# YuePanEdward/MULLS

Measured on NVIDIA H100. Metric: scan-pair registrations/sec (120k-pt 64-beam), higher is better.
Workload: dtype f32 geometry / f64 accumulation

## Files before the change

### mulls_b200/csrc/device_types.cuh

```cuda
#pragma once
#include <cstdint>
#include <cuda_runtime.h>

#include "../../include/mulls_b200/abi.h"
#include "search_core.cuh"

namespace mulls {

constexpr int kNumClasses = MULLS_NUM_CLASSES;
constexpr int kNumSegs = 2 * kNumClasses;
constexpr int kIterBlock = 128;
constexpr int kIngestBlock = 256;
constexpr int kTerms = 28;
constexpr int kMaxLevels = 12;
constexpr int kCoordBits = 12;
constexpr int kDedupMinSrc = 500;
constexpr unsigned kClaimFree = 0x7f7f7f7fu;
constexpr int kIterFlags = 256;

enum PairStatus : int { kRunning = 0, kNeedPosterior = 1, kDone = 2 };

struct ChunkDesc {
    uint32_t pair;
    uint32_t seg;
// ... 18 lines not shown
    int normal_shooting;
    int keep_less;
    uint32_t random_seed;
    double cos_thre;
    double sigma_thre;
    double init[16];
    double tbound[6];
    uint32_t in_off[kNumSegs];
    const float4 *in_ptr[kNumSegs];
    uint32_t in_n[kNumSegs];
    uint32_t in_fmt[kNumSegs];
    uint32_t tgt_base[kNumClasses];
    uint32_t src_base[kNumClasses];
    uint32_t chunk_begin;
    uint32_t chunk_end;
    uint32_t class_chunk_begin[kNumClasses + 1];
    uint32_t src_index_base[kNumClasses];
    uint32_t src_global_n[kNumClasses];
    int sharded;
};

struct PairState {
    double T_total[16];
    double T_inc[16];
    double x[6];
    double cofactor[36];
    double info[36];
    double sigma2;
    double ibb[6];
    float thre;
    float confidence;
    float origin[3];
    float h0, inv_h0;
    int n_levels;
    int status, code, iter, iters_entered, final_buf;
    int source_feature_points_count;
    int n_src[kNumClasses];
    int n_src_g[kNumClasses];
    int n_src_g_next[kNumClasses];
    int n_tgt[kNumClasses];
    uint32_t n_corr[kNumClasses];
    uint32_t n_corr_last[kNumClasses];
    uint32_t seg_count[kNumSegs];
    uint32_t seg_start[kNumSegs];
    uint32_t hash_entries[kNumClasses];
    uint32_t hash_base[kNumClasses];
    uint32_t hash_mask[kNumClasses];
    int bb_src[6];
    int bb_tgt[6];
    uint64_t alg_bytes;
    int kl_keep[kNumSegs];
    uint32_t kl_rank[kNumSegs];
    uint64_t kl_prefix[kNumSegs];
    uint32_t kl_hist[kNumSegs][256];
};

struct LoopCtl {
    int it;
    int n_it_chunks;
    int n_pairs;
    int trace_on;
    int max_iter;
    unsigned solved;
    unsigned n_live[2];
    unsigned work[4];
};

struct DeviceArrays {
    const float4 *in_aos;
    uint64_t *keys_a, *keys_b;
    uint32_t *vals_a, *vals_b;
    float4 *tgt_pos, *tgt_nrm;
    float4 *src_pos[2], *src_nrm[2];
    int *src_prevj[2];
    float4 *src_cert[2];
    int *nn_idx;
    float *nn_d2;
    uint8_t *flags;
    int *corr_j;
    float *corr_w;
    unsigned *claim;
    HashEntry *hash;
    uint32_t hash_pool_entries;
    uint32_t *hash_used;
    uint32_t *blk_kept;
    double *partials;
    double *post_partials;
    PairConst *pc;
    PairState *ps;
    ChunkDesc *in_chunks;
    ChunkDesc *it_chunks;
    mulls_icp_trace *trace;
    int *xch_i32;
    double *xch_f64;
    LoopCtl *ctl;
    uint32_t *live_chunks;
    uint32_t live_stride;
    int *running;
    volatile int *h_running;
    volatile int *h_running_iter;
};

}
```

### mulls_b200/csrc/grid_key.cuh

```cuda
#pragma once
#include <cstdint>

#ifdef __CUDACC__
#define MULLS_HD __host__ __device__ __forceinline__
#else
#define MULLS_HD inline
#endif

namespace mulls {

constexpr uint32_t kKeyHiMask = 0xffffu;

MULLS_HD float flann_l2(float px, float py, float pz, float qx, float qy, float qz) {
    const float dx = px - qx, dy = py - qy, dz = pz - qz;
    return (dx * dx + dy * dy) + dz * dz;
}

MULLS_HD uint32_t cell_key_lo(uint32_t x, uint32_t y, uint32_t z) { return x | (y << 12) | ((z & 0xffu) << 24); }
MULLS_HD uint32_t cell_key_hi(uint32_t z, int level) { return (z >> 8) | ((uint32_t)(level + 1) << 4); }

MULLS_HD uint32_t cell_hash(uint32_t klo, uint32_t khi) {
    uint32_t h = klo * 0x9E3779B1u;
    h ^= khi * 0x85EBCA77u;
    h ^= h >> 15;
    h *= 0x2C1B3C6Du;
    h ^= h >> 13;
    return h;
}

MULLS_HD uint64_t spread12(uint32_t v) {
    uint64_t x = v & 0xfffu;
    x = (x | (x << 16)) & 0x0000ff0000ffull;
    x = (x | (x << 8)) & 0x00f00f00f00full;
    x = (x | (x << 4)) & 0x0c30c30c30c3ull;
    x = (x | (x << 2)) & 0x249249249249ull;
    return x;
}
MULLS_HD uint64_t morton36(uint32_t x, uint32_t y, uint32_t z) { return spread12(x) | (spread12(y) << 1) | (spread12(z) << 2); }

MULLS_HD uint32_t compact12(uint64_t m) {
    uint64_t x = m & 0x249249249249ull;
    x = (x | (x >> 2)) & 0x0c30c30c30c3ull;
    x = (x | (x >> 4)) & 0x00f00f00f00full;
    x = (x | (x >> 8)) & 0x0000ff0000ffull;
    x = (x | (x >> 16)) & 0x00000000ffffull;
    return (uint32_t)x & 0xfffu;
}

}
```

### mulls_b200/csrc/kernels_ingest.cuh

```cuda
#pragma once
#include "device_math.cuh"
#include "device_types.cuh"

namespace mulls {

template <bool kUndistort, bool kNormals>
__device__ __forceinline__ void load_input_point(const PairConst &pc, uint32_t seg, uint32_t local, float4 &pos, float4 &nrm) {
    const bool is_src = seg >= kNumClasses;
    const int cls = seg % kNumClasses;
    const bool undistort = kUndistort && is_src && pc.undistort && cls != MULLS_VERTEX;
    float x, y, z, intensity = 0.0f, curvature = 0.0f;
    float nx = 0.0f, ny = 0.0f, nz = 0.0f;
    const uint32_t fmt = pc.in_fmt[seg];
    if (fmt == 0u) {
        const float4 *in = pc.in_ptr[seg] + 3 * (size_t)local;
        const float4 a = in[0];
        x = a.x, y = a.y, z = a.z;
        if (kNormals) {
            const float4 b = in[1];
            const float4 c = in[2];
            nx = b.x, ny = b.y, nz = b.z;
            intensity = c.x, curvature = c.y;
        } else if (undistort) {
            curvature = reinterpret_cast<const float *>(in + 2)[1];
// ... 96 lines not shown
        tmin[d] = (double)ordered_to_float(ps.bb_tgt[d]);
        tmax[d] = (double)ordered_to_float(ps.bb_tgt[3 + d]);
    }
    const double big = 1.7976931348623157e308;
    double gmin[3], gmax[3];
    if (pc.apply_filter) {
        const float pad = 1.0f;
        for (int d = 0; d < 3; ++d) {
            double lo = (pc.tbound[d] > smin[d]) ? pc.tbound[d] : smin[d];
            double hi = (pc.tbound[3 + d] < smax[d]) ? pc.tbound[3 + d] : smax[d];
            ps.ibb[d] = lo - (double)pad;
            ps.ibb[3 + d] = hi + (double)pad;
            gmin[d] = fmax(tmin[d], ps.ibb[d]);
            gmax[d] = fmin(tmax[d], ps.ibb[3 + d]);
        }
    } else {
        for (int d = 0; d < 3; ++d) {
            ps.ibb[d] = -big;
            ps.ibb[3 + d] = big;
            gmin[d] = tmin[d];
            gmax[d] = tmax[d];
        }
    }
    double ext = 0.0;
    for (int d = 0; d < 3; ++d) {
        if (!(gmax[d] >= gmin[d])) {
            gmin[d] = 0.0;
            gmax[d] = 0.0;
        }
        ext = fmax(ext, gmax[d] - gmin[d]);
    }
    const int ncell = 1 << kCoordBits;
    float h0 = kH0Min;
    while ((ext + 8.0 * h0) * 1.001 > (double)h0 * (ncell - 4)) h0 *= 2.0f;
    ps.h0 = h0;
    ps.inv_h0 = 1.0f / h0;
    for (int d = 0; d < 3; ++d) ps.origin[d] = (float)gmin[d] - 2.0f * h0;
    const float rmax = 2.5f * pc.thre_unit * 1.0001f;
    int L = 2;
    while (L < kMaxLevels && 0.999f * 0.5f * h0 * (float)(1 << (L - 1)) < rmax) ++L;
    if (pc.normal_shooting) L = kMaxLevels;
    ps.n_levels = L;

    for (int i = 0; i < 16; ++i) {
        ps.T_total[i] = pc.init[i];
        ps.T_inc[i] = (i % 5 == 0) ? 1.0 : 0.0;
    }
    for (int i = 0; i < 36; ++i) ps.cofactor[i] = ps.info[i] = (i % 7 == 0) ? 1.0 : 0.0;
    for (int i = 0; i < 6; ++i) ps.x[i] = 0.0;
    ps.sigma2 = 1.0;
    ps.thre = pc.thre_unit;
    ps.confidence = 1.0f;
    ps.status = kRunning;
    ps.code = 0;
    ps.iter = 0;
    ps.iters_entered = 0;
    ps.final_buf = 0;
    ps.alg_bytes = 0;
    if (pc.max_iter <= 0) {
        ps.status = kDone;
        const int left = atomicSub(A.running, 1) - 1;
        *A.h_running = left;
        __threadfence_system();
    }
}

template <bool kUndistort, bool kFiniteOnly = false>
__global__ void __launch_bounds__(kIngestBlock) k_make_keys(DeviceArrays A) {
    const ChunkDesc cd = A.in_chunks[blockIdx.x];
    const PairConst &pc = A.pc[cd.pair];
    PairState &ps = A.ps[cd.pair];
    const uint32_t seg = cd.seg;
    const uint32_t local = cd.first + threadIdx.x;
    const bool valid = local < pc.in_n[seg];
    bool inside = false;
    if (valid) {
        const size_t gi = (size_t)pc.in_off[seg] + local;
        float4 p, unused;
        load_input_point<kUndistort, false>(pc, seg, local, p, unused);
        const double *b = ps.ibb;
        inside = (double)p.x > b[0] && (double)p.x < b[3] && (double)p.y > b[1] && (double)p.y < b[4] &&
                 (double)p.z > b[2] && (double)p.z < b[5];
        if (kFiniteOnly) inside = inside && finite_xyz(p);
        uint64_t key = ~0ull;
        if (inside) {
            const int hi = (1 << kCoordBits) - 1;
            int cx = (int)floorf((p.x - ps.origin[0]) * ps.inv_h0);
            int cy = (int)floorf((p.y - ps.origin[1]) * ps.inv_h0);
            int cz = (int)floorf((p.z - ps.origin[2]) * ps.inv_h0);
            cx = min(max(cx, 0), hi);
            cy = min(max(cy, 0), hi);
            cz = min(max(cz, 0), hi);
            key = ((uint64_t)(cd.pair * kNumSegs + seg) << 36) | morton36((uint32_t)cx, (uint32_t)cy, (uint32_t)cz);
        }
        A.keys_a[gi] = key;
        A.vals_a[gi] = (uint32_t)gi;
    }
    const unsigned ballot = __ballot_sync(0xffffffffu, inside);
    if ((threadIdx.x & 31) == 0 && ballot) atomicAdd(&ps.seg_count[seg], (unsigned)__popc(ballot));
}

__device__ __forceinline__ uint64_t sample_key(uint32_t seed, uint32_t cloud_id, uint32_t index) {
    uint64_t z = (((uint64_t)seed << 40) ^ ((uint64_t)cloud_id << 32) ^ (uint64_t)index) + 0x9e3779b97f4a7c15ull;
    z = (z ^ (z >> 30)) * 0xbf58476d1ce4e5b9ull;
    z = (z ^ (z >> 27)) * 0x94d049bb133111ebull;
    return z ^ (z >> 31);
}

__global__ void k_keepless_plan(DeviceArrays A, int n_pairs) {
    const int p = blockIdx.x * blockDim.x + threadIdx.x;
    if (p >= n_pairs) return;
    const PairConst &pc = A.pc[p];
    PairState &ps = A.ps[p];
    for (int s = 0; s < kNumSegs; ++s) {
        ps.kl_keep[s] = -1;
        ps.kl_prefix[s] = 0;
        ps.kl_rank[s] = 0;
        for (int b = 0; b < 256; ++b) ps.kl_hist[s][b] = 0;
    }
    if (!pc.keep_less) return;
    const int S = kNumClasses;
    auto plan = [&](int seg, int keep) {
        if ((int)ps.seg_count[seg] > keep) {
            ps.kl_keep[seg] = keep;
            ps.kl_rank[seg] = (uint32_t)keep;
        }
        return ((int)ps.seg_count[seg] > keep) ? keep : (int)ps.seg_count[seg];
    };
    const int tg = plan(MULLS_GROUND, (int)(ps.seg_count[MULLS_GROUND] / 2));
    const int tf = plan(MULLS_FACADE, (int)(ps.seg_count[MULLS_FACADE] / 2));
    plan(S + MULLS_GROUND, tg / 4);
    plan(S + MULLS_FACADE, tf / 2);
    plan(S + MULLS_PILLAR, (int)ps.seg_count[MULLS_PILLAR]);
    plan(S + MULLS_BEAM, (int)ps.seg_count[MULLS_BEAM]);
    plan(S + MULLS_ROOF, (int)ps.seg_count[MULLS_ROOF]);
    plan(S + MULLS_VERTEX, (int)ps.seg_count[MULLS_VERTEX]);
}

__global__ void __launch_bounds__(kIngestBlock) k_keepless_hist(DeviceArrays A, int pass) {
    const ChunkDesc cd = A.in_chunks[blockIdx.x];
    const PairConst &pc = A.pc[cd.pair];
    PairState &ps = A.ps[cd.pair];
    const uint32_t seg = cd.seg;
    if (ps.kl_keep[seg] <= 0) return;
    __shared__ uint32_t s_hist[256];
    s_hist[threadIdx.x] = 0;
    __syncthreads();
    const uint32_t local = cd.first + threadIdx.x;
    if (local < pc.in_n[seg]) {
        const size_t gi = (size_t)pc.in_off[seg] + local;
        if (A.keys_a[gi] != ~0ull) {
            const uint64_t key = sample_key(pc.random_seed, seg, local);
            const int shift = 56 - 8 * pass;
            const bool match = (pass == 0) || ((key >> (shift + 8)) == (ps.kl_prefix[seg] >> (shift + 8)));
            if (match) atomicAdd(&s_hist[(key >> shift) & 0xff], 1u);
        }
    }
    __syncthreads();
    if (s_hist[threadIdx.x]) atomicAdd(&ps.kl_hist[seg][threadIdx.x], s_hist[threadIdx.x]);
}

__global__ void k_keepless_step(DeviceArrays A, int n_pairs, int pass) {
    const int p = blockIdx.x * blockDim.x + threadIdx.x;
    if (p >= n_pairs) return;
    PairState &ps = A.ps[p];
    for (int s = 0; s < kNumSegs; ++s) {
        if (ps.kl_keep[s] <= 0) continue;
        uint32_t cum = 0, rank = ps.kl_rank[s];
        int d = 0;
        for (; d < 256; ++d) {
            const uint32_t h = ps.kl_hist[s][d];
            if (cum + h >= rank) break;
            cum += h;
        }
        ps.kl_prefix[s] |= (uint64_t)d << (56 - 8 * pass);
        ps.kl_rank[s] = rank - cum;
        for (int b = 0; b < 256; ++b) ps.kl_hist[s][b] = 0;
    }
}

__global__ void __launch_bounds__(kIngestBlock) k_keepless_mark(DeviceArrays A) {
    const ChunkDesc cd = A.in_chunks[blockIdx.x];
    const PairConst &pc = A.pc[cd.pair];
    PairState &ps = A.ps[cd.pair];
    const uint32_t seg = cd.seg;
    const int keep = ps.kl_keep[seg];
    if (keep < 0) return;
    const uint32_t local = cd.first + threadIdx.x;
    bool drop = false;
    if (local < pc.in_n[seg]) {
        const size_t gi = (size_t)pc.in_off[seg] + local;
        if (A.keys_a[gi] != ~0ull) {
            drop = (keep == 0) || sample_key(pc.random_seed, seg, local) > ps.kl_prefix[seg];
            if (drop) A.keys_a[gi] = ~0ull;
        }
    }
    const unsigned b = __ballot_sync(0xffffffffu, drop);
    if ((threadIdx.x & 31) == 0 && b) atomicSub(&ps.seg_count[seg], (unsigned)__popc(b));
}

__global__ void k_seg_offsets(DeviceArrays A, int n_pairs) {
    __shared__ uint32_t carry;
    __shared__ uint32_t warp_sums[32];
    if (threadIdx.x == 0) carry = 0;
    __syncthreads();
    const int total = n_pairs * kNumSegs;
    for (int base = 0; base < total; base += blockDim.x) {
        const int i = base + threadIdx.x;
        uint32_t v = 0;
        if (i < total) v = A.ps[i / kNumSegs].seg_count[i % kNumSegs];
        uint32_t incl = v;
        for (int o = 1; o < 32; o <<= 1) {
            uint32_t t = __shfl_up_sync(0xffffffffu, incl, o);
            if ((threadIdx.x & 31) >= o) incl += t;
        }
        if ((threadIdx.x & 31) == 31) warp_sums[threadIdx.x >> 5] = incl;
        __syncthreads();
        if (threadIdx.x < 32) {
            uint32_t w = (threadIdx.x < (blockDim.x >> 5)) ? warp_sums[threadIdx.x] : 0;
            uint32_t wi = w;
            for (int o = 1; o < 32; o <<= 1) {
                uint32_t t = __shfl_up_sync(0xffffffffu, wi, o);
                if (threadIdx.x >= o) wi += t;
            }
            warp_sums[threadIdx.x] = wi - w;
        }
        __syncthreads();
        const uint32_t excl = carry + warp_sums[threadIdx.x >> 5] + incl - v;
        if (i < total) A.ps[i / kNumSegs].seg_start[i % kNumSegs] = excl;
        __syncthreads();
        if (threadIdx.x == blockDim.x - 1) carry = excl + v;
        __syncthreads();
    }
    for (int p = threadIdx.x; p < n_pairs; p += blockDim.x) {
        PairState &ps = A.ps[p];
        const PairConst &pc = A.pc[p];
        for (int c = 0; c < kNumClasses; ++c) {
            ps.n_tgt[c] = (int)ps.seg_count[c];
            ps.n_src[c] = (int)ps.seg_count[kNumClasses + c];
            ps.n_src_g[c] = ps.n_src[c];
            ps.n_corr[c] = 0;
            ps.n_corr_last[c] = 0;
        }
        int cnt = 0;
        if (pc.used[MULLS_PILLAR]) cnt += ps.n_src[MULLS_PILLAR];
        if (pc.used[MULLS_FACADE]) cnt += ps.n_src[MULLS_FACADE];
        if (pc.used[MULLS_BEAM]) cnt += ps.n_src[MULLS_BEAM];
        ps.source_feature_points_count = cnt;
    }
}

__device__ __forceinline__ int cell_top(const uint64_t *keys, uint32_t i, uint64_t kcur) {
    if (kcur == ~0ull || ((uint32_t)(kcur >> 36) % kNumSegs) >= kNumClasses) return -1;
    if (i == 0) return kMaxLevels - 1;
    const uint64_t kprev = keys[i - 1];
    if ((kprev >> 36) != (kcur >> 36)) return kMaxLevels - 1;
    const uint64_t diff = (kcur ^ kprev) & ((1ull << 36) - 1);
    if (diff == 0) return -1;
    return (63 - __clzll((long long)diff)) / 3;
}

template <bool kUndistort>
__global__ void __launch_bounds__(256) k_gather(DeviceArrays A, const uint64_t *keys, const uint32_t *vals, uint32_t n_total) {
    const uint32_t i = blockIdx.x * blockDim.x + threadIdx.x;
    const uint64_t key = i < n_total ? keys[i] : ~0ull;
    const uint32_t sg = (uint32_t)(key >> 36);
    const uint32_t pair = sg / kNumSegs, seg = sg % kNumSegs;
    const int top = cell_top(keys, i, key);
    const int cnt = top < 0 ? 0 : min(top, A.ps[pair].n_levels - 1) + 1;
    const bool is_tgt = key != ~0ull && seg < kNumClasses;
    const unsigned grp = __match_any_sync(0xffffffffu, is_tgt ? sg : 0xffffffffu);
    if (grp == 0xffffffffu) {
        const int tot = __reduce_add_sync(0xffffffffu, cnt);
        if ((threadIdx.x & 31) == 0 && tot > 0) atomicAdd(&A.ps[pair].hash_entries[seg], (unsigned)tot);
    } else if (cnt > 0) {
        atomicAdd(&A.ps[pair].hash_entries[seg], (unsigned)cnt);
    }
    if (key == ~0ull) return;
    const PairConst &pc = A.pc[pair];
    float4 pos, nrm;
    load_input_point<kUndistort, true>(pc, seg, vals[i] - pc.in_off[seg], pos, nrm);
    const uint32_t local = i - A.ps[pair].seg_start[seg];
    if (seg < kNumClasses) {
        const uint32_t d = pc.tgt_base[seg] + local;
        A.tgt_pos[d] = pos;
        A.tgt_nrm[d] = nrm;
    } else {
        const uint32_t d = pc.src_base[seg - kNumClasses] + local;
        if (pc.sharded) nrm.w = __int_as_float(__float_as_int(nrm.w) + (int)pc.src_index_base[seg - kNumClasses]);
        A.src_pos[0][d] = pos;
        A.src_nrm[0][d] = nrm;
        A.src_prevj[0][d] = -1;
        A.src_cert[0][d] = make_float4(0.f, 0.f, 0.f, 0.f);
    }
}

__device__ __forceinline__ void hash_insert(HashEntry *table, uint32_t hmask, uint32_t klo, uint32_t khi, uint32_t children,
                                            uint32_t start, uint32_t count) {
    uint32_t slot = cell_hash(klo, khi) & hmask;
    const unsigned long long packed = (unsigned long long)klo | ((unsigned long long)(khi | (children << 16)) << 32);
    while (true) {
        unsigned long long *kp = reinterpret_cast<unsigned long long *>(&table[slot]);
        if (atomicCAS(kp, 0ull, packed) == 0ull) {
            *reinterpret_cast<uint2 *>(&table[slot].start) = make_uint2(start, count);
            return;
        }
        slot = (slot + 1) & hmask;
    }
}

__device__ __forceinline__ uint32_t cell_end(const uint64_t *keys, uint32_t b, uint32_t hi, uint64_t p, int shift) {
    uint32_t in = b, out = hi, step = 1;
    while (in + step < hi) {
        if ((keys[in + step] >> shift) != p) {
            out = in + step;
            break;
        }
        in += step;
        step <<= 1;
    }
    while (out - in > 1) {
        const uint32_t mid = in + (out - in) / 2;
        if ((keys[mid] >> shift) == p) in = mid;
        else out = mid;
    }
    return out;
}

__global__ void __launch_bounds__(256) k_hash_build(DeviceArrays A, const uint64_t *keys, uint32_t n_total) {
    const uint32_t i = blockIdx.x * blockDim.x + threadIdx.x;
    if (i >= n_total || A.hash_used[1]) return;
    const uint64_t kcur = keys[i];
    const int top = cell_top(keys, i, kcur);
    if (top < 0) return;
    const uint32_t sg = (uint32_t)(kcur >> 36);
    const uint32_t pair = sg / kNumSegs, cls = sg % kNumSegs;
    const PairState &ps = A.ps[pair];
    const int L = ps.n_levels;
    const uint32_t seg_begin = ps.seg_start[cls], seg_end = seg_begin + ps.seg_count[cls];
    HashEntry *table = A.hash + ps.hash_base[cls];
    const uint32_t hmask = ps.hash_mask[cls];
    const uint64_t m = kcur & ((1ull << 36) - 1);
    const uint32_t x0 = compact12(m), y0 = compact12(m >> 1), z0 = compact12(m >> 2);
    uint32_t end = cell_end(keys, i, seg_end, kcur, 0);
    for (int l = 0; l <= top && l < L; ++l) {
        uint32_t children = 0;
        if (l > 0) {
            const int shift = 3 * l;
            const uint64_t p = kcur >> shift;
            children = 1u << ((kcur >> (shift - 3)) & 7u);
            while (end < seg_end) {
                const uint64_t k = keys[end];
                if ((k >> shift) != p) break;
                children |= 1u << ((k >> (shift - 3)) & 7u);
                end = cell_end(keys, end, seg_end, k >> (shift - 3), shift - 3);
            }
        }
        const uint32_t x = x0 >> l, y = y0 >> l, z = z0 >> l;
        hash_insert(table, hmask, cell_key_lo(x, y, z), cell_key_hi(z, l), children, i - seg_begin, end - i);
    }
}

constexpr uint64_t kHashSlack = 4;
__device__ __forceinline__ uint64_t hash_table_cap(int attempt, uint32_t cells) {
    const uint64_t want = (attempt == 0) ? kHashSlack * cells : (attempt == 1) ? 2ull * cells : (5ull * cells) / 4 + 1;
    uint64_t cap = 16;
    while (cap < want) cap <<= 1;
    return cap;
}
__global__ void k_hash_layout(DeviceArrays A, int n_pairs) {
    if (threadIdx.x != 0 || blockIdx.x != 0) return;
    for (int attempt = 0; attempt < 3; ++attempt) {
        uint64_t used = 0;
        bool overflow = false;
        for (int p = 0; p < n_pairs && !overflow; ++p) {
            PairState &ps = A.ps[p];
            for (int c = 0; c < kNumClasses; ++c) {
                const uint64_t cap = hash_table_cap(attempt, ps.hash_entries[c]);
                if (used + cap > A.hash_pool_entries) {
                    overflow = true;
                    break;
                }
                ps.hash_base[c] = (uint32_t)used;
                ps.hash_mask[c] = (uint32_t)(cap - 1);
                used += cap;
            }
        }
        A.hash_used[0] = overflow ? 0u : (uint32_t)used;
        A.hash_used[1] = overflow ? 1u : 0u;
        if (!overflow) return;
    }
    uint64_t need = 0;
    for (int p = 0; p < n_pairs; ++p) {
        PairState &ps = A.ps[p];
        for (int c = 0; c < kNumClasses; ++c) {
            need += hash_table_cap(2, ps.hash_entries[c]);
            ps.hash_base[c] = 0;
            ps.hash_mask[c] = 0;
        }
        if (ps.status == kRunning) {
            ps.status = kDone;
            *A.h_running = atomicSub(A.running, 1) - 1;
        }
    }
    __threadfence_system();
    A.hash_used[2] = need < 0xffffffffull ? (uint32_t)need : 0xffffffffu;
}

__global__ void __launch_bounds__(256) k_hash_clear(DeviceArrays A) {
    const uint32_t used = A.hash_used[0];
    const uint4 z = make_uint4(0, 0, 0, 0);
    for (uint32_t i = blockIdx.x * blockDim.x + threadIdx.x; i < used; i += gridDim.x * blockDim.x)
        reinterpret_cast<uint4 *>(A.hash)[i] = z;
}

}
```

### mulls_b200/csrc/mulls_b200.cu

```cuda
#include <algorithm>
#include <atomic>
#include <memory>
#include <cmath>
#include <cstdio>
#include <chrono>
#include <cstring>
#include <string>
#include <vector>

#include <cub/device/device_radix_sort.cuh>
#include <cub/device/device_scan.cuh>
#include <cub/device/device_select.cuh>

#include <dlfcn.h>
#include <mutex>

#include "device_types.cuh"
#include "host_pack.h"
#include "scan_io.h"
#include "kernels_ingest.cuh"
#include "kernels_iterate.cuh"
#include "kernels_pca.cuh"
#include "kernels_map.cuh"
#include "kernels_classify.cuh"
// ... 250 lines not shown
        mulls_destroy(ctx);
        return nullptr;
    };
    if ((e = cudaSetDevice(device)) != cudaSuccess) return fail("cudaSetDevice", e);
    if ((e = cudaStreamCreateWithFlags(&ctx->stream, cudaStreamNonBlocking)) != cudaSuccess) return fail("stream", e);
    const size_t cs = ctx->cap_src = max_pairs * max_src_pts;
    const size_t ct = ctx->cap_tgt = max_pairs * max_tgt_pts;
    const size_t cin = ctx->cap_in = cs + ct;
    if (cin >= (1ull << 31)) {
        g_create_error = "mulls_create: more than 2^31 points per context";
        mulls_destroy(ctx);
        return nullptr;
    }
    ctx->cap_it_chunks = ceil_div(cs, kIterBlock) + max_pairs * (kNumClasses + 1);
    ctx->cap_in_chunks = ceil_div(cin, kIngestBlock) + max_pairs * kNumSegs;
    DeviceArrays &A = ctx->A;
    float4 *in = nullptr;
#define ALLOC(ptr, n)                                                   \
    if ((e = dev_alloc(ctx, &(ptr), (n))) != cudaSuccess) return fail(#ptr, e)
    ALLOC(in, 3 * cin);
    A.in_aos = in;
    ALLOC(A.keys_a, cin);
    ALLOC(A.keys_b, cin);
    ALLOC(A.vals_a, cin);
    ALLOC(A.vals_b, cin);
    ALLOC(A.tgt_pos, ct + kScanOverrun);
    ALLOC(A.tgt_nrm, ct);
    for (int b = 0; b < 2; ++b) {
        ALLOC(A.src_pos[b], cs);
        ALLOC(A.src_nrm[b], cs);
        ALLOC(A.src_prevj[b], cs);
        ALLOC(A.src_cert[b], cs);
    }
    ALLOC(A.nn_idx, cs);
    ALLOC(A.nn_d2, cs);
    ALLOC(A.flags, cs);
    ALLOC(A.corr_j, cs);
    ALLOC(A.corr_w, cs);
    ALLOC(A.claim, ct);
    {
        size_t pool = 12 * ct + 64 * max_pairs * kNumClasses;
        if (pool >= (1ull << 32)) pool = (1ull << 32) - 1;
        A.hash_pool_entries = (uint32_t)pool;
        ALLOC(A.hash, pool);
    }
    ALLOC(A.hash_used, 3);
    ALLOC(A.ctl, 1);
    ALLOC(A.blk_kept, ctx->cap_it_chunks);
    ALLOC(A.partials, ctx->cap_it_chunks * kTerms);
    ALLOC(A.post_partials, ctx->cap_it_chunks * 2);
    ALLOC(A.pc, max_pairs);
    ALLOC(A.ps, max_pairs);
    ALLOC(A.in_chunks, ctx->cap_in_chunks);
    ALLOC(A.it_chunks, ctx->cap_it_chunks);
    ALLOC(A.live_chunks, 2 * ctx->cap_it_chunks);
    A.live_stride = (uint32_t)ctx->cap_it_chunks;
    {
        int sms = 0;
        if (cudaDeviceGetAttribute(&sms, cudaDevAttrMultiProcessorCount, device) != cudaSuccess || sms <= 0) sms = 132;
        ctx->num_sms = sms;
    }
    ALLOC(ctx->d_results, max_pairs + ceil_div(max_pairs * sizeof(uint64_t), sizeof(mulls_icp_result)) + 1);
    ALLOC(ctx->d_trace, max_pairs);
    ALLOC(A.running, 1);
    ALLOC(A.xch_i32, 32);
    ALLOC(A.xch_f64, kNumClasses * kTerms + 8);
#undef ALLOC
    if ((e = cudaHostAlloc((void **)&ctx->h_running, (1 + kIterFlags) * sizeof(int), cudaHostAllocMapped)) != cudaSuccess)
        return fail("mapped flag", e);
    {
        int *dptr = nullptr;
        if ((e = cudaHostGetDevicePointer((void **)&dptr, ctx->h_running, 0)) != cudaSuccess) return fail("mapped flag", e);
        A.h_running = dptr;
        A.h_running_iter = dptr + 1;
    }
    ctx->ev_done.resize(MULLS_MAX_TRACE_ITERS);
    for (auto &ev : ctx->ev_done) cudaEventCreateWithFlags(&ev, cudaEventDisableTiming);
    A.trace = ctx->d_trace;
    if ((e = cudaMallocHost((void **)&ctx->h_results, max_pairs * (sizeof(mulls_icp_result) + sizeof(uint64_t)))) != cudaSuccess)
        return fail("pinned results", e);
    if ((e = cudaMallocHost((void **)&ctx->h_flags, 4 * sizeof(uint32_t))) != cudaSuccess) return fail("pinned flags", e);
    if ((e = cudaMallocHost((void **)&ctx->h_ctl, sizeof(LoopCtl))) != cudaSuccess) return fail("pinned control block", e);
    {
        size_t bytes = 0;
        cub::DeviceRadixSort::SortPairs(nullptr, bytes, A.keys_a, A.keys_b, A.vals_a, A.vals_b, (int)cin, 0, 64,
                                        ctx->stream);
        ctx->cub_temp_bytes = bytes;
        if ((e = cudaMalloc(&ctx->cub_temp, std::max<size_t>(bytes, 16))) != cudaSuccess) return fail("cub temp", e);
    }
    cudaEventCreate(&ctx->ev_begin);
    cudaEventCreate(&ctx->ev_ingest);
    cudaEventCreate(&ctx->ev_iter);
    cudaEventCreate(&ctx->ev_end);
    cudaEventCreate(&ctx->ev_h2d0);
    ctx->ev_search.resize(2 * MULLS_MAX_TRACE_ITERS);
    for (auto &ev : ctx->ev_search) cudaEventCreate(&ev);
    if ((e = cudaMemsetAsync(A.ps, 0, max_pairs * sizeof(PairState), ctx->stream)) != cudaSuccess) return fail("memset", e);
    if ((e = cudaStreamSynchronize(ctx->stream)) != cudaSuccess) return fail("sync", e);
    return ctx;
}

int mulls_set_tunable(mulls_ctx *ctx, const char *name, int value) {
    if (!ctx || !name) return MULLS_E_ARG;
    if (ctx->twin) {
        const int rc = mulls_set_tunable(ctx->twin, name, value);
        if (rc != MULLS_OK) return rc;
    }
    std::string n(name);
    if (n == "use_graph") ctx->use_graph = value;
    else if (n == "host_pack") ctx->host_pack = value;
    else if (n == "pack_threads") PackPool::get().ensure_workers(value);
    else return MULLS_E_ARG;
    return MULLS_OK;
}

int mulls_pack_rows(const float *aos48, size_t n, int format, float *out) {
    if ((n > 0 && (!aos48 || !out)) || (format != kFmtPacked28 && format != kFmtPacked32) || ((uintptr_t)out % 16) != 0)
        return MULLS_E_ARG;
    pack_rows(aos48, 0, n, format, out, out + 4 * n);
    _mm_sfence();
    return MULLS_OK;
}

static int io_code(int rc) {
    switch (rc) {
    case mulls_io::kOk: return MULLS_OK;
    case mulls_io::kArg: return MULLS_E_ARG;
    case mulls_io::kCapacity: return MULLS_E_CAPACITY;
    case mulls_io::kUnsupported: return MULLS_E_UNSUPPORTED;
    default: return MULLS_E_IO;
    }
}
int mulls_scan_probe(const char *path, size_t *n_points) { return io_code(mulls_io::probe_scan(path, n_points)); }
int mulls_scan_read(const char *path, float *rows48, size_t capacity_points, size_t *n_points, double local_bound[6],
                    int normalize_intensity) {
    return io_code(mulls_io::read_scan(path, rows48, capacity_points, n_points, local_bound, normalize_intensity));
}
int mulls_pose_write(const char *path, const double pose[16], int overwrite) {
    return io_code(mulls_io::append_pose(path, pose, overwrite));
}
void *mulls_host_alloc(size_t bytes) {
    void *p = nullptr;
    if (cudaHostAlloc(&p, bytes ? bytes : 1, cudaHostAllocDefault) != cudaSuccess) {
        cudaGetLastError();
        return nullptr;
    }
    return p;
}
void mulls_host_free(void *p) {
    if (p) cudaFreeHost(p);
}

int mulls_get_stats(const mulls_ctx *ctx, mulls_run_stats *out) {
    if (!ctx || !out) return MULLS_E_ARG;
    *out = ctx->stats;
    return MULLS_OK;
}

static SlerpConst slerp_const_of(const double *T) {
    SlerpConst sc;
    double *q = sc.q;
    double t = T[0] + T[5] + T[10];
    if (t > 0.0) {
        t = std::sqrt(t + 1.0);
        q[3] = 0.5 * t;
        t = 0.5 / t;
        q[0] = (T[9] - T[6]) * t;
        q[1] = (T[2] - T[8]) * t;
        q[2] = (T[4] - T[1]) * t;
// ... 214 lines not shown
        if (ce == cudaSuccess && !ctx->h_it_chunks.empty())
            ce = cudaMemcpyAsync(ctx->A.it_chunks, ctx->h_it_chunks.data(), ctx->h_it_chunks.size() * sizeof(ChunkDesc),
                                 cudaMemcpyHostToDevice, ctx->stream);
        tables_sent = true;
        if (ce == cudaSuccess && cudaEventRecord(ctx->ev_h2d0, ctx->stream) == cudaSuccess) ctx->h2d_timed = true;
        const double t_pack0 = wall_ms();
        for (size_t p = 0; p < n_pairs; ++p) {
            pool.help_until_done(pending[p]);
            if (p + 1 == n_pairs) ctx->up_ms_pack = (float)(wall_ms() - t_pack0);
            const size_t b = slot_begin[p], e = slot_begin[p + 1];
            if (e > b && ce == cudaSuccess)
                ce = cudaMemcpyAsync((void *)(ctx->A.in_aos + b), ctx->h_stage + b, (e - b) * sizeof(float4), cudaMemcpyHostToDevice,
                                     ctx->stream);
        }
        CK(ce);
    } else {
    if (cudaEventRecord(ctx->ev_h2d0, ctx->stream) == cudaSuccess) ctx->h2d_timed = true;
    for (size_t p = 0; p < n_pairs; ++p) {
        PairConst &pc = ctx->h_pc[p];
        for (int s = 0; s < kNumSegs; ++s) {
            const mulls_cloud_view &v = (s < kNumClasses) ? tgt[p * kNumClasses + s] : src[p * kNumClasses + (s - kNumClasses)];
            pc.in_ptr[s] = ctx->A.in_aos + 3 * (size_t)pc.in_off[s];
            pc.in_fmt[s] = kFmtRows48;
            if (v.n == 0) continue;
            if (tgt_on_device && s < kNumClasses) {
                pc.in_ptr[s] = (const float4 *)v.aos48;
                continue;
            }
            CK(cudaMemcpyAsync((void *)(ctx->A.in_aos + 3 * (size_t)pc.in_off[s]), v.aos48, v.n * 48, cudaMemcpyHostToDevice,
                               ctx->stream));
        }
    }
    }
    if (!tables_sent) {
        CK(cudaMemcpyAsync(ctx->A.pc, ctx->h_pc.data(), n_pairs * sizeof(PairConst), cudaMemcpyHostToDevice, ctx->stream));
        if (!ctx->h_in_chunks.empty())
            CK(cudaMemcpyAsync(ctx->A.in_chunks, ctx->h_in_chunks.data(), ctx->h_in_chunks.size() * sizeof(ChunkDesc),
                               cudaMemcpyHostToDevice, ctx->stream));
        if (!ctx->h_it_chunks.empty())
            CK(cudaMemcpyAsync(ctx->A.it_chunks, ctx->h_it_chunks.data(), ctx->h_it_chunks.size() * sizeof(ChunkDesc),
                               cudaMemcpyHostToDevice, ctx->stream));
    }
    if (resident) CK(cudaStreamSynchronize(ctx->stream));
    ctx->n_pairs = n_pairs;
    ctx->n_in = in_off;
    ctx->n_src_total = s_off;
    ctx->n_tgt_total = t_off;
    ctx->max_iter_max = max_iter_max;
    ctx->any_keep_less = any_keep_less;
    ctx->any_normal_shooting = any_shoot;
    ctx->any_undistort = any_undistort;
    ctx->uploaded = true;
    ctx->up_ms_host = (float)(wall_ms() - t_up0);
    return MULLS_OK;
}

static int launch_ingest(mulls_ctx *ctx, DeviceArrays &A, bool trace, uint64_t &launches, mulls_allreduce_fn hook = nullptr,
                         void *user = nullptr, bool finite_only = false) {
    cudaStream_t st = ctx->stream;
    const int np = (int)ctx->n_pairs;
    const uint32_t n_in = (uint32_t)ctx->n_in;
    if (trace) CK(cudaMemsetAsync(ctx->d_trace, 0, np * sizeof(mulls_icp_trace), st));
    CK(cudaMemsetAsync(A.claim, 0x7f, std::max<size_t>(ctx->n_tgt_total, 1) * sizeof(unsigned), st));
    k_state_init<<<(unsigned)ceil_div(np, 128), 128, 0, st>>>(A, np);
    ++launches;
    const unsigned n_inc = (unsigned)ctx->h_in_chunks.size();
    if (n_inc) {
        if (ctx->any_undistort) k_ingest_bbox<true><<<n_inc, kIngestBlock, 0, st>>>(A);
        else if (finite_only) k_ingest_bbox<false, true><<<n_inc, kIngestBlock, 0, st>>>(A);
        else k_ingest_bbox<false><<<n_inc, kIngestBlock, 0, st>>>(A);
        ++launches;
    }
    if (hook) {
        k_shard_pack_setup<<<1, 1, 0, st>>>(A, 0);
        if (hook(user, A.xch_i32, 6, 1, 1, (void *)st) != 0) {
            ctx->err = "all-reduce callback failed";
            return MULLS_E_COMM;
        }
        k_shard_pack_setup<<<1, 1, 0, st>>>(A, 1);
        launches += 2;
    }
    k_pair_setup<<<(unsigned)ceil_div(np, 128), 128, 0, st>>>(A, np);
    ++launches;
    if (n_inc) {
        if (ctx->any_undistort) k_make_keys<true><<<n_inc, kIngestBlock, 0, st>>>(A);
        else if (finite_only) k_make_keys<false, true><<<n_inc, kIngestBlock, 0, st>>>(A);
        else k_make_keys<false><<<n_inc, kIngestBlock, 0, st>>>(A);
        ++launches;
        if (ctx->any_keep_less) {
            const unsigned pb = (unsigned)ceil_div(np, 64);
            k_keepless_plan<<<pb, 64, 0, st>>>(A, np);
            for (int pass = 0; pass < 8; ++pass) {
                k_keepless_hist<<<n_inc, kIngestBlock, 0, st>>>(A, pass);
                k_keepless_step<<<pb, 64, 0, st>>>(A, np, pass);
            }
            k_keepless_mark<<<n_inc, kIngestBlock, 0, st>>>(A);
            launches += 18;
        }
        int seg_bits = 1;
        while ((1ull << seg_bits) <= (uint64_t)np * kNumSegs) ++seg_bits;
        size_t bytes = ctx->cub_temp_bytes;
        CK(cub::DeviceRadixSort::SortPairs(ctx->cub_temp, bytes, A.keys_a, A.keys_b, A.vals_a, A.vals_b, (int)n_in, 0,
                                           36 + seg_bits, st));
    }
    k_seg_offsets<<<1, 256, 0, st>>>(A, np);
    ++launches;
    if (hook) {
        k_shard_pack_setup<<<1, 1, 0, st>>>(A, 2);
        if (hook(user, A.xch_i32, kNumClasses, 1, 0, (void *)st) != 0) {
            ctx->err = "all-reduce callback failed";
            return MULLS_E_COMM;
        }
        k_shard_pack_setup<<<1, 1, 0, st>>>(A, 3);
        launches += 2;
    }
    if (n_in) {
        const unsigned nb = (unsigned)ceil_div(n_in, 256);
        if (ctx->any_undistort) k_gather<true><<<nb, 256, 0, st>>>(A, A.keys_b, A.vals_b, n_in);
        else k_gather<false><<<nb, 256, 0, st>>>(A, A.keys_b, A.vals_b, n_in);
        k_hash_layout<<<1, 32, 0, st>>>(A, np);
        k_hash_clear<<<1184, 256, 0, st>>>(A);
        k_hash_build<<<nb, 256, 0, st>>>(A, A.keys_b, n_in);
        launches += 4;
    } else {
        k_hash_layout<<<1, 32, 0, st>>>(A, np);
        ++launches;
    }
    return MULLS_OK;
}

static unsigned chunk_bucket(const mulls_ctx *ctx) {
    unsigned b = 1;
    while (b < (unsigned)ctx->h_it_chunks.size()) b <<= 1;
    return b;
}
static unsigned resident_grid(const mulls_ctx *ctx, int blocks_per_sm) {
    return std::min((unsigned)(ctx->num_sms * blocks_per_sm), chunk_bucket(ctx));
}
static void launch_search(mulls_ctx *ctx, cudaStream_t st, const DeviceArrays &A, int buf, int it) {
    const unsigned grid = resident_grid(ctx, kSearchBlocksPerSm);
    const int mode = it < 0 ? -1 : (it >= kKeepFromIter ? 2 : (it == kKeepFromIter - 1 ? 1 : 0));
    if (mode < 0 || mode == 0) k_search<0><<<grid, kIterBlock, 0, st>>>(A, buf, it);
    if (mode < 0 || mode == 1) k_search<1><<<grid, kIterBlock, 0, st>>>(A, buf, it);
    if (mode < 0 || mode == 2) k_search<2><<<grid, kIterBlock, 0, st>>>(A, buf, it);
}
constexpr int kShootBlocksPerSm = 8, kResolveBlocksPerSm = 16, kAccumulateBlocksPerSm = 8;
constexpr int kPollPause = 64;

static int build_iteration_graph(mulls_ctx *ctx) {
    const int key[2] = {(int)chunk_bucket(ctx), ctx->any_normal_shooting ? 1 : 0};
    if (ctx->graph_exec && std::memcmp(key, ctx->graph_key, sizeof(key)) == 0) return MULLS_OK;
    if (ctx->graph_exec) cudaGraphExecDestroy(ctx->graph_exec), ctx->graph_exec = nullptr;
    if (ctx->graph) cudaGraphDestroy(ctx->graph), ctx->graph = nullptr;
    cudaStream_t st = ctx->stream;
    DeviceArrays A = ctx->A;
    const unsigned cap_chunks = (unsigned)std::max<size_t>(ctx->cap_it_chunks, 1), cap_pairs = (unsigned)std::max<size_t>(ctx->max_pairs, 1);
    CK(cudaGraphCreate(&ctx->graph, 0));
    cudaGraphConditionalHandle handle;
    CK(cudaGraphConditionalHandleCreate(&handle, ctx->graph, 1, cudaGraphCondAssignDefault));
    cudaGraphNodeParams wp = {cudaGraphNodeTypeConditional};
    wp.conditional.handle = handle;
    wp.conditional.type = cudaGraphCondTypeWhile;
    wp.conditional.size = 1;
    cudaGraphNode_t while_node;
    CK(cudaGraphAddNode(&while_node, ctx->graph, nullptr, 0, &wp));
    cudaGraph_t body = wp.conditional.phGraph_out[0];
    CK(cudaStreamBeginCaptureToGraph(st, body, nullptr, nullptr, 0, cudaStreamCaptureModeThreadLocal));
    launch_search(ctx, st, A, -1, -1);
    if (ctx->any_normal_shooting)
        k_search_shoot<<<resident_grid(ctx, kShootBlocksPerSm), kIterBlock, 0, st>>>(A, -1);
    k_resolve<<<resident_grid(ctx, kResolveBlocksPerSm), kIterBlock, 0, st>>>(A, -1);
    k_accumulate<<<resident_grid(ctx, kAccumulateBlocksPerSm), kIterBlock, 0, st>>>(A, -1);
    k_solve<<<cap_pairs, kSolveThreads, 0, st>>>(A, -1, (unsigned long long)handle);
    CK(cudaStreamEndCapture(st, nullptr));
    CK(cudaStreamBeginCaptureToGraph(st, ctx->graph, &while_node, nullptr, 1, cudaStreamCaptureModeThreadLocal));
    k_posterior<<<std::min(cap_chunks, chunk_bucket(ctx)), kIterBlock, 0, st>>>(A);
    k_finalize<<<(unsigned)ceil_div(cap_pairs, 64), 64, 0, st>>>(A, -1);
    k_collect<<<(unsigned)ceil_div(cap_pairs, 128), 128, 0, st>>>(A, -1, ctx->d_results);
    CK(cudaStreamEndCapture(st, nullptr));
    CK(cudaGraphInstantiate(&ctx->graph_exec, ctx->graph, 0));
    std::memcpy(ctx->graph_key, key, sizeof(key));
    return MULLS_OK;
}

static int grow_hash_pool(mulls_ctx *ctx) {
    const uint32_t need = ctx->h_flags[2];
    DeviceArrays &A = ctx->A;
    if (need <= A.hash_pool_entries || need == 0xffffffffu) {
        ctx->err = "hash pool exhausted (the target clouds need " + std::to_string(need) + " grid entries)";
        return MULLS_E_CAPACITY;
    }
    HashEntry *fresh = nullptr;
    if (cudaMalloc(&fresh, (size_t)need * sizeof(HashEntry)) != cudaSuccess) {
        cudaGetLastError();
        ctx->err = "hash pool exhausted, and no device memory to grow it to " + std::to_string(need) + " entries";
        return MULLS_E_CAPACITY;
    }
    std::replace(ctx->allocs.begin(), ctx->allocs.end(), (void *)A.hash, (void *)fresh);
    CK(cudaFree(A.hash));
    A.hash = fresh;
    A.hash_pool_entries = need;
    if (ctx->graph_exec) cudaGraphExecDestroy(ctx->graph_exec), ctx->graph_exec = nullptr;
    if (ctx->graph) cudaGraphDestroy(ctx->graph), ctx->graph = nullptr;
    return MULLS_OK;
}

static int run_impl_inner(mulls_ctx *ctx, mulls_icp_result *out, mulls_icp_trace *trace, mulls_allreduce_fn hook, void *user,
                          bool finish_now);
// ... 1853 lines not shown
```

Measured before the change: 6241.

## Pack point index into sort key and parallelize hash table layout

Packs the per-segment local point index into the low bits of the 64-bit radix sort key, so ingest can use a keys-only sort over the upper bits instead of sorting key/value pairs. This removes the value array traffic from the sort and from key generation. It falls back to pair sort when the bits don't fit. The hash layout kernel also becomes a 512-thread block prefix sum instead of a single-thread serial loop over all tables.

```diff
diff --git a/mulls_b200/csrc/device_types.cuh b/mulls_b200/csrc/device_types.cuh
--- a/mulls_b200/csrc/device_types.cuh
+++ b/mulls_b200/csrc/device_types.cuh
@@ -124,6 +124,7 @@
     unsigned *claim;
     HashEntry *hash;
     uint32_t hash_pool_entries;
+    int key_idx_bits;
     uint32_t *hash_used;
     uint32_t *blk_kept;
     double *partials;
diff --git a/mulls_b200/csrc/grid_key.cuh b/mulls_b200/csrc/grid_key.cuh
--- a/mulls_b200/csrc/grid_key.cuh
+++ b/mulls_b200/csrc/grid_key.cuh
@@ -47,4 +47,24 @@
     return (uint32_t)x & 0xfffu;
 }
 
+constexpr int kMortonKeyBits = 36;
+constexpr uint64_t kSortKeyNone = ~0ull;
+
+MULLS_HD uint64_t sort_key_pack(uint32_t seg_id, uint64_t morton, uint32_t local, int idx_bits) {
+    return ((((uint64_t)seg_id << kMortonKeyBits) | morton) << idx_bits) | (local & ((1ull << idx_bits) - 1));
 }
+MULLS_HD uint32_t sort_key_seg(uint64_t key, int idx_bits) { return (uint32_t)(key >> (kMortonKeyBits + idx_bits)); }
+MULLS_HD uint64_t sort_key_morton(uint64_t key, int idx_bits) { return (key >> idx_bits) & ((1ull << kMortonKeyBits) - 1); }
+MULLS_HD uint32_t sort_key_local(uint64_t key, int idx_bits) { return (uint32_t)(key & ((1ull << idx_bits) - 1)); }
+MULLS_HD uint64_t sort_key_cell(uint64_t key, int idx_bits, int level) { return key >> (idx_bits + 3 * level); }
+MULLS_HD int sort_key_top_level(uint64_t a, uint64_t b, int idx_bits) {
+    const uint64_t diff = sort_key_morton(a ^ b, idx_bits);
+    if (diff == 0) return -1;
+#ifdef __CUDA_ARCH__
+    return (63 - __clzll((long long)diff)) / 3;
+#else
+    return (63 - __builtin_clzll(diff)) / 3;
+#endif
+}
+
+}
diff --git a/mulls_b200/csrc/kernels_ingest.cuh b/mulls_b200/csrc/kernels_ingest.cuh
--- a/mulls_b200/csrc/kernels_ingest.cuh
+++ b/mulls_b200/csrc/kernels_ingest.cuh
@@ -202,7 +202,7 @@
         inside = (double)p.x > b[0] && (double)p.x < b[3] && (double)p.y > b[1] && (double)p.y < b[4] &&
                  (double)p.z > b[2] && (double)p.z < b[5];
         if (kFiniteOnly) inside = inside && finite_xyz(p);
-        uint64_t key = ~0ull;
+        uint64_t key = kSortKeyNone;
         if (inside) {
             const int hi = (1 << kCoordBits) - 1;
             int cx = (int)floorf((p.x - ps.origin[0]) * ps.inv_h0);
@@ -211,10 +211,11 @@
             cx = min(max(cx, 0), hi);
             cy = min(max(cy, 0), hi);
             cz = min(max(cz, 0), hi);
-            key = ((uint64_t)(cd.pair * kNumSegs + seg) << 36) | morton36((uint32_t)cx, (uint32_t)cy, (uint32_t)cz);
+            key = sort_key_pack(cd.pair * kNumSegs + seg, morton36((uint32_t)cx, (uint32_t)cy, (uint32_t)cz), local,
+                                A.key_idx_bits);
         }
         A.keys_a[gi] = key;
-        A.vals_a[gi] = (uint32_t)gi;
+        if (A.key_idx_bits == 0) A.vals_a[gi] = (uint32_t)gi;
     }
     const unsigned ballot = __ballot_sync(0xffffffffu, inside);
     if ((threadIdx.x & 31) == 0 && ballot) atomicAdd(&ps.seg_count[seg], (unsigned)__popc(ballot));
@@ -269,7 +270,7 @@
     const uint32_t local = cd.first + threadIdx.x;
     if (local < pc.in_n[seg]) {
         const size_t gi = (size_t)pc.in_off[seg] + local;
-        if (A.keys_a[gi] != ~0ull) {
+        if (A.keys_a[gi] != kSortKeyNone) {
             const uint64_t key = sample_key(pc.random_seed, seg, local);
             const int shift = 56 - 8 * pass;
             const bool match = (pass == 0) || ((key >> (shift + 8)) == (ps.kl_prefix[seg] >> (shift + 8)));
@@ -310,9 +311,9 @@
     bool drop = false;
     if (local < pc.in_n[seg]) {
         const size_t gi = (size_t)pc.in_off[seg] + local;
-        if (A.keys_a[gi] != ~0ull) {
+        if (A.keys_a[gi] != kSortKeyNone) {
             drop = (keep == 0) || sample_key(pc.random_seed, seg, local) > ps.kl_prefix[seg];
-            if (drop) A.keys_a[gi] = ~0ull;
+            if (drop) A.keys_a[gi] = kSortKeyNone;
         }
     }
     const unsigned b = __ballot_sync(0xffffffffu, drop);
@@ -370,25 +371,24 @@
     }
 }
 
-__device__ __forceinline__ int cell_top(const uint64_t *keys, uint32_t i, uint64_t kcur) {
-    if (kcur == ~0ull || ((uint32_t)(kcur >> 36) % kNumSegs) >= kNumClasses) return -1;
+__device__ __forceinline__ int cell_top(const uint64_t *keys, uint32_t i, uint64_t kcur, int idx_bits) {
+    if (kcur == kSortKeyNone || sort_key_seg(kcur, idx_bits) % kNumSegs >= kNumClasses) return -1;
     if (i == 0) return kMaxLevels - 1;
     const uint64_t kprev = keys[i - 1];
-    if ((kprev >> 36) != (kcur >> 36)) return kMaxLevels - 1;
-    const uint64_t diff = (kcur ^ kprev) & ((1ull << 36) - 1);
-    if (diff == 0) return -1;
-    return (63 - __clzll((long long)diff)) / 3;
+    if (sort_key_seg(kprev, idx_bits) != sort_key_seg(kcur, idx_bits)) return kMaxLevels - 1;
+    return sort_key_top_level(kprev, kcur, idx_bits);
 }
 
 template <bool kUndistort>
 __global__ void __launch_bounds__(256) k_gather(DeviceArrays A, const uint64_t *keys, const uint32_t *vals, uint32_t n_total) {
     const uint32_t i = blockIdx.x * blockDim.x + threadIdx.x;
-    const uint64_t key = i < n_total ? keys[i] : ~0ull;
-    const uint32_t sg = (uint32_t)(key >> 36);
+    const int ib = A.key_idx_bits;
+    const uint64_t key = i < n_total ? keys[i] : kSortKeyNone;
+    const uint32_t sg = sort_key_seg(key, ib);
     const uint32_t pair = sg / kNumSegs, seg = sg % kNumSegs;
-    const int top = cell_top(keys, i, key);
+    const int top = cell_top(keys, i, key, ib);
     const int cnt = top < 0 ? 0 : min(top, A.ps[pair].n_levels - 1) + 1;
-    const bool is_tgt = key != ~0ull && seg < kNumClasses;
+    const bool is_tgt = key != kSortKeyNone && seg < kNumClasses;
     const unsigned grp = __match_any_sync(0xffffffffu, is_tgt ? sg : 0xffffffffu);
     if (grp == 0xffffffffu) {
         const int tot = __reduce_add_sync(0xffffffffu, cnt);
@@ -396,10 +396,10 @@
     } else if (cnt > 0) {
         atomicAdd(&A.ps[pair].hash_entries[seg], (unsigned)cnt);
     }
-    if (key == ~0ull) return;
+    if (key == kSortKeyNone) return;
     const PairConst &pc = A.pc[pair];
     float4 pos, nrm;
-    load_input_point<kUndistort, true>(pc, seg, vals[i] - pc.in_off[seg], pos, nrm);
+    load_input_point<kUndistort, true>(pc, seg, ib ? sort_key_local(key, ib) : vals[i] - pc.in_off[seg], pos, nrm);
     const uint32_t local = i - A.ps[pair].seg_start[seg];
     if (seg < kNumClasses) {
         const uint32_t d = pc.tgt_base[seg] + local;
@@ -429,10 +429,10 @@
     }
 }
 
-__device__ __forceinline__ uint32_t cell_end(const uint64_t *keys, uint32_t b, uint32_t hi, uint64_t p, int shift) {
+__device__ __forceinline__ uint32_t cell_end(const uint64_t *keys, uint32_t b, uint32_t hi, uint64_t p, int idx_bits, int level) {
     uint32_t in = b, out = hi, step = 1;
     while (in + step < hi) {
-        if ((keys[in + step] >> shift) != p) {
+        if (sort_key_cell(keys[in + step], idx_bits, level) != p) {
             out = in + step;
             break;
         }
@@ -441,7 +441,7 @@
     }
     while (out - in > 1) {
         const uint32_t mid = in + (out - in) / 2;
-        if ((keys[mid] >> shift) == p) in = mid;
+        if (sort_key_cell(keys[mid], idx_bits, level) == p) in = mid;
         else out = mid;
     }
     return out;
@@ -450,30 +450,31 @@
 __global__ void __launch_bounds__(256) k_hash_build(DeviceArrays A, const uint64_t *keys, uint32_t n_total) {
     const uint32_t i = blockIdx.x * blockDim.x + threadIdx.x;
     if (i >= n_total || A.hash_used[1]) return;
+    const int ib = A.key_idx_bits;
     const uint64_t kcur = keys[i];
-    const int top = cell_top(keys, i, kcur);
+    const int top = cell_top(keys, i, kcur, ib);
     if (top < 0) return;
-    const uint32_t sg = (uint32_t)(kcur >> 36);
+    const uint32_t sg = sort_key_seg(kcur, ib);
     const uint32_t pair = sg / kNumSegs, cls = sg % kNumSegs;
     const PairState &ps = A.ps[pair];
     const int L = ps.n_levels;
     const uint32_t seg_begin = ps.seg_start[cls], seg_end = seg_begin + ps.seg_count[cls];
     HashEntry *table = A.hash + ps.hash_base[cls];
     const uint32_t hmask = ps.hash_mask[cls];
-    const uint64_t m = kcur & ((1ull << 36) - 1);
+    const uint64_t m = sort_key_morton(kcur, ib);
     const uint32_t x0 = compact12(m), y0 = compact12(m >> 1), z0 = compact12(m >> 2);
-    uint32_t end = cell_end(keys, i, seg_end, kcur, 0);
+    uint32_t end = cell_end(keys, i, seg_end, sort_key_cell(kcur, ib, 0), ib, 0);
     for (int l = 0; l <= top && l < L; ++l) {
         uint32_t children = 0;
         if (l > 0) {
-            const int shift = 3 * l;
-            const uint64_t p = kcur >> shift;
-            children = 1u << ((kcur >> (shift - 3)) & 7u);
+            const uint64_t p = sort_key_cell(kcur, ib, l);
+            children = 1u << (sort_key_cell(kcur, ib, l - 1) & 7u);
             while (end < seg_end) {
                 const uint64_t k = keys[end];
-                if ((k >> shift) != p) break;
-                children |= 1u << ((k >> (shift - 3)) & 7u);
-                end = cell_end(keys, end, seg_end, k >> (shift - 3), shift - 3);
+                if (sort_key_cell(k, ib, l) != p) break;
+                const uint64_t child = sort_key_cell(k, ib, l - 1);
+                children |= 1u << (child & 7u);
+                end = cell_end(keys, end, seg_end, child, ib, l - 1);
             }
         }
         const uint32_t x = x0 >> l, y = y0 >> l, z = z0 >> l;
@@ -488,43 +489,76 @@
     while (cap < want) cap <<= 1;
     return cap;
 }
+__device__ __forceinline__ uint64_t block_exclusive_sum(uint64_t v, uint64_t &total) {
+    __shared__ uint64_t warp_sums[32];
+    __shared__ uint64_t block_sum;
+    const unsigned lane = threadIdx.x & 31, warp = threadIdx.x >> 5;
+    uint64_t incl = v;
+    for (int o = 1; o < 32; o <<= 1) {
+        const uint64_t t = __shfl_up_sync(0xffffffffu, incl, o);
+        if (lane >= o) incl += t;
+    }
+    __syncthreads();
+    if (lane == 31) warp_sums[warp] = incl;
+    __syncthreads();
+    if (warp == 0) {
+        const uint64_t w = lane < (blockDim.x >> 5) ? warp_sums[lane] : 0;
+        uint64_t wi = w;
+        for (int o = 1; o < 32; o <<= 1) {
+            const uint64_t t = __shfl_up_sync(0xffffffffu, wi, o);
+            if (lane >= o) wi += t;
+        }
+        warp_sums[lane] = wi - w;
+        if (lane == 31) block_sum = wi;
+    }
+    __syncthreads();
+    total = block_sum;
+    return warp_sums[warp] + incl - v;
+}
+constexpr int kLayoutThreads = 512;
 __global__ void k_hash_layout(DeviceArrays A, int n_pairs) {
-    if (threadIdx.x != 0 || blockIdx.x != 0) return;
+    if (blockIdx.x != 0) return;
+    const uint32_t tables = (uint32_t)n_pairs * kNumClasses;
+    uint64_t used = 0;
     for (int attempt = 0; attempt < 3; ++attempt) {
-        uint64_t used = 0;
-        bool overflow = false;
-        for (int p = 0; p < n_pairs && !overflow; ++p) {
-            PairState &ps = A.ps[p];
-            for (int c = 0; c < kNumClasses; ++c) {
-                const uint64_t cap = hash_table_cap(attempt, ps.hash_entries[c]);
-                if (used + cap > A.hash_pool_entries) {
-                    overflow = true;
-                    break;
-                }
-                ps.hash_base[c] = (uint32_t)used;
+        used = 0;
+        for (uint32_t first = 0; first < tables; first += blockDim.x) {
+            const uint32_t t = first + threadIdx.x;
+            PairState &ps = A.ps[t < tables ? t / kNumClasses : 0];
+            const int c = t % kNumClasses;
+            const uint64_t cap = t < tables ? hash_table_cap(attempt, ps.hash_entries[c]) : 0;
+            uint64_t sum;
+            const uint64_t base = used + block_exclusive_sum(cap, sum);
+            if (t < tables && base + cap <= A.hash_pool_entries) {
+                ps.hash_base[c] = (uint32_t)base;
                 ps.hash_mask[c] = (uint32_t)(cap - 1);
-                used += cap;
-            }
-        }
-        A.hash_used[0] = overflow ? 0u : (uint32_t)used;
-        A.hash_used[1] = overflow ? 1u : 0u;
-        if (!overflow) return;
-    }
-    uint64_t need = 0;
+            }
+            used += sum;
+        }
+        if (used <= A.hash_pool_entries) {
+            if (threadIdx.x == 0) {
+                A.hash_used[0] = (uint32_t)used;
+                A.hash_used[1] = 0u;
+            }
+            return;
+        }
+    }
+    for (uint32_t t = threadIdx.x; t < tables; t += blockDim.x) {
+        A.ps[t / kNumClasses].hash_base[t % kNumClasses] = 0;
+        A.ps[t / kNumClasses].hash_mask[t % kNumClasses] = 0;
+    }
+    if (threadIdx.x != 0) return;
     for (int p = 0; p < n_pairs; ++p) {
         PairState &ps = A.ps[p];
-        for (int c = 0; c < kNumClasses; ++c) {
-            need += hash_table_cap(2, ps.hash_entries[c]);
-            ps.hash_base[c] = 0;
-            ps.hash_mask[c] = 0;
-        }
         if (ps.status == kRunning) {
             ps.status = kDone;
             *A.h_running = atomicSub(A.running, 1) - 1;
         }
     }
+    A.hash_used[0] = 0u;
+    A.hash_used[1] = 1u;
     __threadfence_system();
-    A.hash_used[2] = need < 0xffffffffull ? (uint32_t)need : 0xffffffffu;
+    A.hash_used[2] = used < 0xffffffffull ? (uint32_t)used : 0xffffffffu;
 }
 
 __global__ void __launch_bounds__(256) k_hash_clear(DeviceArrays A) {
diff --git a/mulls_b200/csrc/mulls_b200.cu b/mulls_b200/csrc/mulls_b200.cu
--- a/mulls_b200/csrc/mulls_b200.cu
+++ b/mulls_b200/csrc/mulls_b200.cu
@@ -356,9 +356,11 @@
     if ((e = cudaMallocHost((void **)&ctx->h_flags, 4 * sizeof(uint32_t))) != cudaSuccess) return fail("pinned flags", e);
     if ((e = cudaMallocHost((void **)&ctx->h_ctl, sizeof(LoopCtl))) != cudaSuccess) return fail("pinned control block", e);
     {
-        size_t bytes = 0;
+        size_t bytes = 0, keys_bytes = 0;
         cub::DeviceRadixSort::SortPairs(nullptr, bytes, A.keys_a, A.keys_b, A.vals_a, A.vals_b, (int)cin, 0, 64,
                                         ctx->stream);
+        cub::DeviceRadixSort::SortKeys(nullptr, keys_bytes, A.keys_a, A.keys_b, (int)cin, 0, 64, ctx->stream);
+        bytes = std::max(bytes, keys_bytes);
         ctx->cub_temp_bytes = bytes;
         if ((e = cudaMalloc(&ctx->cub_temp, std::max<size_t>(bytes, 16))) != cudaSuccess) return fail("cub temp", e);
     }
@@ -739,6 +741,15 @@
     }
     k_pair_setup<<<(unsigned)ceil_div(np, 128), 128, 0, st>>>(A, np);
     ++launches;
+    int seg_bits = 1;
+    while ((1ull << seg_bits) <= (uint64_t)np * kNumSegs) ++seg_bits;
+    uint32_t max_n = 1;
+    for (int p = 0; p < np; ++p)
+        for (int s = 0; s < kNumSegs; ++s) max_n = std::max(max_n, ctx->h_pc[p].in_n[s]);
+    int idx_bits = 1;
+    while ((1ull << idx_bits) < max_n) ++idx_bits;
+    if (idx_bits + kMortonKeyBits + seg_bits > 64) idx_bits = 0;
+    A.key_idx_bits = idx_bits;
     if (n_inc) {
         if (ctx->any_undistort) k_make_keys<true><<<n_inc, kIngestBlock, 0, st>>>(A);
         else if (finite_only) k_make_keys<false, true><<<n_inc, kIngestBlock, 0, st>>>(A);
@@ -754,11 +765,11 @@
             k_keepless_mark<<<n_inc, kIngestBlock, 0, st>>>(A);
             launches += 18;
         }
-        int seg_bits = 1;
-        while ((1ull << seg_bits) <= (uint64_t)np * kNumSegs) ++seg_bits;
         size_t bytes = ctx->cub_temp_bytes;
-        CK(cub::DeviceRadixSort::SortPairs(ctx->cub_temp, bytes, A.keys_a, A.keys_b, A.vals_a, A.vals_b, (int)n_in, 0,
-                                           36 + seg_bits, st));
+        const int end_bit = idx_bits + kMortonKeyBits + seg_bits;
+        if (idx_bits) CK(cub::DeviceRadixSort::SortKeys(ctx->cub_temp, bytes, A.keys_a, A.keys_b, (int)n_in, idx_bits, end_bit, st));
+        else CK(cub::DeviceRadixSort::SortPairs(ctx->cub_temp, bytes, A.keys_a, A.keys_b, A.vals_a, A.vals_b, (int)n_in, 0,
+                                                end_bit, st));
     }
     k_seg_offsets<<<1, 256, 0, st>>>(A, np);
     ++launches;
@@ -775,12 +786,12 @@
         const unsigned nb = (unsigned)ceil_div(n_in, 256);
         if (ctx->any_undistort) k_gather<true><<<nb, 256, 0, st>>>(A, A.keys_b, A.vals_b, n_in);
         else k_gather<false><<<nb, 256, 0, st>>>(A, A.keys_b, A.vals_b, n_in);
-        k_hash_layout<<<1, 32, 0, st>>>(A, np);
+        k_hash_layout<<<1, kLayoutThreads, 0, st>>>(A, np);
         k_hash_clear<<<1184, 256, 0, st>>>(A);
         k_hash_build<<<nb, 256, 0, st>>>(A, A.keys_b, n_in);
         launches += 4;
     } else {
-        k_hash_layout<<<1, 32, 0, st>>>(A, np);
+        k_hash_layout<<<1, kLayoutThreads, 0, st>>>(A, np);
         ++launches;
     }
     return MULLS_OK;
```

New measurement: 6374 (median of 6 runs). 1.02x the previous value.
